# flo-stilz/Audio-Key-Estimation

Hardware: AMD Instinct MI355X
Metric: clips/s (15 s @ 22.05 kHz), HIP CQT + PitchClassNet forward (higher is better)
Workload: dtype f32 accumulation everywhere; pitch / semitone / layer-0 convolutions: f16 activations x f16 weights (per-channel power-of-two scaled) on MFMA, one product; last layer's pitch-class convolutions and heads: 3-term split-bf16 on MFMA (hi*hi + lo*hi + hi*lo); CQT filter bank: 3-term split-bf16 on MFMA

## Files before the change

audio-key-estimation_amd/csrc/pcnet.hip:

```cpp
#include <algorithm>
#include <cmath>
#include <cstdlib>
#include <cstring>
#include <map>
#include <string>
#include <vector>

#include "common.h"
#include "pcnet_kernels.h"
#include "pcnet_bwd_kernels.h"

using namespace ake_k;

namespace {

constexpr double kBnEps = 1e-5;
constexpr size_t kLdsBudget = 64 * 1024;
constexpr size_t kBfFragsPerConv = 14 * 2 * 64 + 64;

struct TensorSpec {
    std::string name;
    int64_t shape[4];
    int ndim;
};
// ... 412 lines not shown
    a.Tp = p2p_pitch(a.J);
    a.R = std::max(1, std::min(H, 8 * kP2pMT * 16 / a.J));
    auto lds_of = [&](int R) { return (static_cast<size_t>(R + 6) * a.Tp + (kP2pStreamB ? 0 : kBfFragsPerConv)) * sizeof(uint4); };
    while (a.R > 1 && lds_of(a.R) > 76 * 1024) --a.R;
    AKE_REQUIRE(lds_of(a.R) <= 150 * 1024, AKE_ERR_UNSUPPORTED, "conv %s: %d frames do not fit the bf16 kernel's LDS patch", name, T);
    a.n_row_tiles = (H + a.R - 1) / a.R;
    static ake::DeviceOnce attr_set;
    if (attr_set.need()) {
        AKE_HIP_CHECK(hipFuncSetAttribute(reinterpret_cast<const void*>(conv_p2p_f16_kernel<true, false>), hipFuncAttributeMaxDynamicSharedMemorySize, 150 * 1024));
        AKE_HIP_CHECK(hipFuncSetAttribute(reinterpret_cast<const void*>(conv_p2p_f16_kernel<false, false>), hipFuncAttributeMaxDynamicSharedMemorySize, 150 * 1024));
        AKE_HIP_CHECK(hipFuncSetAttribute(reinterpret_cast<const void*>(conv_p2p_f16_kernel<true, true>), hipFuncAttributeMaxDynamicSharedMemorySize, 150 * 1024));
        attr_set.mark();
    }
    dim3 grid(a.n_row_tiles, 1, batch), block(512);
    ake::ProfScope ps(name, s);
    AKE_REQUIRE(!nchw || oh, AKE_ERR_STATE, "conv %s: the assembling variant writes channels-last planes", name);
    if (nchw) hipLaunchKernelGGL((conv_p2p_f16_kernel<true, true>), grid, block, lds_of(a.R), s, a);
    else if (oh) hipLaunchKernelGGL((conv_p2p_f16_kernel<true, false>), grid, block, lds_of(a.R), s, a);
    else hipLaunchKernelGGL((conv_p2p_f16_kernel<false, false>), grid, block, lds_of(a.R), s, a);
    return AKE_OK;
}

int g_keep_taps = 0;

int device_cus() {
    static int n_cus = 0;
    if (!n_cus) {
        int dev = 0;
        if (hipGetDevice(&dev) != hipSuccess || hipDeviceGetAttribute(&n_cus, hipDeviceAttributeMultiprocessorCount, dev) != hipSuccess) n_cus = -1;
    }
    return n_cus;
}

int p2p_ps_rows(int H, int T, bool semi, int* plane_pos, size_t* lds) {
    if (T < 2 || (T & 1) || device_cus() < 8) return 0;
    const int J = T / 2, Tp = p2p_pitch(J);
    auto plane_of = [&](int R) { return ((R + 6) * Tp + 63) / 64 * 64; };
    auto lds_of = [&](int R) { return (static_cast<size_t>(2) * plane_of(R) + (semi ? 2 * 8 * kP2pMT * 16 * 2 : 8 * kP2pMT * kP2pPsStage)) * sizeof(uint4); };
    int R = std::max(1, std::min(H, 8 * kP2pMT * 16 / J));
    if (semi) R = R / 3 * 3;
    while (R >= (semi ? 3 : 1) && (lds_of(R) > 156 * 1024 || plane_of(R) / 64 > 8 * kP2pPieces)) R -= semi ? 3 : 1;
    if (R < (semi ? 3 : 1) || H < R + 6) return 0;
    if (semi && (H % 3 || (H / 3) % 12)) return 0;
    if (plane_pos) *plane_pos = plane_of(R);
    if (lds) *lds = lds_of(R);
    return R;
}

bool p2p_fuses_semi(const ake_pcnet* n, int i, int P, int T) {
    return !g_keep_taps && !n->cfg.p2pc_conv && !n->cfg.stay_sixth && i == n->cfg.num_layers - 1 && p2p_uses_f16(n, i, T) && static_cast<size_t>(i) < n->semi.size() && n->semi[i].bf_off >= 0 &&
           p2p_ps_rows(P, T, true, nullptr, nullptr) > 0;
}

enum class P2pIn : unsigned char {
    Planes,
    Src,
    SrcFramesMajor,
    SrcF16x4,
};
enum class P2pOut : unsigned char {
    Plane,
    Nchw,
    Semi,
    SemiFold,
};
struct P2pPsIo {
    P2pIn in = P2pIn::Planes;
    const unsigned short* planes = nullptr;
    Src src{};
    P2pOut out = P2pOut::Plane;
    unsigned short* plane = nullptr;
    float* dst = nullptr;
    int dst_ctot = 0;
    int fold_coff = 0;
// ... 61 lines not shown
        }
    }
    a.dst = io.dst; a.dst_clip_stride = static_cast<long long>(io.dst_ctot) * (semi ? H / 3 : H) * T; a.oh = io.plane;
    if (semi) { a.sfrag = n->bf_frags_dev + io.semi->bf_off; a.sbias = n->blob_dev + io.semi->b_off; }
    a.H = H; a.T = T; a.J = T / 2; a.Tp = p2p_pitch(a.J);
    a.n_row_tiles = g.n_row_tiles; a.n_tiles = g.n_tiles;
    if (io.out == P2pOut::SemiFold) {
        a.n_oct = g.n_oct; a.n_units = g.n_units;
        a.dst = io.dst + static_cast<long long>(io.fold_coff) * 12 * T;
        a.dst_clip_stride = static_cast<long long>(io.dst_ctot) * 12 * T;
    }
    static ake::DeviceOnce attr_set;
    if (attr_set.need()) {
        const void* fns[] = {reinterpret_cast<const void*>(conv_p2p_f16_ps_kernel<3, 0>),
                             reinterpret_cast<const void*>(conv_p2p_f16_ps_kernel<1, 0>), reinterpret_cast<const void*>(conv_p2p_f16_ps_kernel<1, 5>),
                             reinterpret_cast<const void*>(conv_p2p_f16_ps_kernel<1, 8>), reinterpret_cast<const void*>(conv_p2p_f16_ps_kernel<0, 0>),
                             reinterpret_cast<const void*>(conv_p2p_f16_ps_kernel<2, 0>), reinterpret_cast<const void*>(conv_p2p_f16_ps_kernel<1, 3>)};
        for (const void* f : fns) AKE_HIP_CHECK(hipFuncSetAttribute(f, hipFuncAttributeMaxDynamicSharedMemorySize, 160 * 1024));
        attr_set.mark();
    }
    dim3 grid(g.grid), block(512);
    ake::ProfScope ps(name, s);
    switch (io.out) {
        case P2pOut::SemiFold: hipLaunchKernelGGL((conv_p2p_f16_ps_kernel<3, 0>), grid, block, g.lds, s, a); break;
        case P2pOut::Semi: hipLaunchKernelGGL((conv_p2p_f16_ps_kernel<2, 0>), grid, block, g.lds, s, a); break;
        case P2pOut::Nchw: hipLaunchKernelGGL((conv_p2p_f16_ps_kernel<0, 0>), grid, block, g.lds, s, a); break;
        case P2pOut::Plane:
            if (io.in == P2pIn::Planes) hipLaunchKernelGGL((conv_p2p_f16_ps_kernel<1, 0>), grid, block, g.lds, s, a);
            else if (io.in == P2pIn::SrcF16x4) hipLaunchKernelGGL((conv_p2p_f16_ps_kernel<1, 3>), grid, block, g.lds, s, a);
            else if (a.c0 + a.c1 <= 5) hipLaunchKernelGGL((conv_p2p_f16_ps_kernel<1, 5>), grid, block, g.lds, s, a);
            else hipLaunchKernelGGL((conv_p2p_f16_ps_kernel<1, 8>), grid, block, g.lds, s, a);
            break;
    }
    return AKE_OK;
}

struct P2pX3Plan {
    bool ok = false;
    int R = 0, plane_pos = 0, n_row_tiles = 0, n_tiles = 0, grid = 0;
    size_t lds = 0;
};
P2pX3Plan p2p_f16x3_plan(int c0, int c1, int cout, int batch, int H, int T, bool dst16) {
    P2pX3Plan g;
    if (T < 2 || (T & 1) || c0 < 1 || c0 + c1 > 8 || cout > 8 || batch < 1) return g;
    const int n_cus = device_cus();
    if (n_cus < 8) return g;
    const int Tp = p2p_pitch(T / 2);
    auto plane_of = [&](int R) { return ((R + 6) * Tp + 63) / 64 * 64; };
    auto lds_of = [&](int R) { return (static_cast<size_t>(4) * plane_of(R) + 8 * kP2pMT * kP2pPsStage) * sizeof(uint4); };
    int R = std::max(1, std::min(H, 8 * kP2pMT * 16 / (T / 2)));
    while (R >= 1 && (lds_of(R) > 156 * 1024 || plane_of(R) > 3 * 512)) --R;
    if (R < 1 || H < R + 6) return g;
    if ((R * T) % 4 || (static_cast<long long>(H) * T) % 4 || (static_cast<long long>(cout) * H * T) % 4 || !dst16) return g;
    g.R = R; g.plane_pos = plane_of(R); g.lds = lds_of(R);
    g.n_row_tiles = (H + R - 1) / R;
    g.n_tiles = g.n_row_tiles * batch;
    g.grid = std::min(n_cus / 8 * 8, (g.n_tiles + 7) / 8 * 8);
    g.ok = true;
    return g;
}

int run_p2p_f16x3(const ake_pcnet* n, const P2pX3Plan& g, long long frag_off, const Src& src, const float* in_aff, const float* bias, int batch, int H, int T,
                  float* dst, int cout, double* stats, int stats_stride, hipStream_t s, const char* name, const unsigned int* in_amax = nullptr, bool lrelu = false) {
    AKE_REQUIRE(g.ok && frag_off >= 0 && src.ctot0 == 0, AKE_ERR_STATE, "conv %s: a convolution that does not qualify was sent to the f16 x 3 persistent kernel", name);
    AKE_REQUIRE(g.n_tiles == g.n_row_tiles * batch, AKE_ERR_STATE, "conv %s: the f16 x 3 persistent kernel was planned for another batch than these %d clips", name, batch);
    AKE_REQUIRE(!(reinterpret_cast<uintptr_t>(dst) & 15), AKE_ERR_STATE, "conv %s: the f16 x 3 persistent kernel was planned for 16-byte stores to an unaligned tensor", name);
// ... 335 lines not shown
            if (h == 2 && !c.genre) break;
            for (int j = 0; j + 1 < c.head_layers; ++j) {
                b->hst[h].push_back(cv.take<float>(hid));
                b->aff_hst[h].push_back(cv.take<float>(3 * 2 * n->final_ch));
            }
            b->g_map[h] = cv.take<float>(B * 12 * b->Tf);
        }
    }
    b->bytes = ake::align_up(cv.off, 256);
    return AKE_OK;
}

enum class L0Form : unsigned char { Generic, FusedValu, FusedMfma };
enum class PStack : unsigned char { Generic, F16x3, F16 };
enum class PcStack : unsigned char { Generic, F16x3, Bf16, Fused };
enum class HeadForm : unsigned char { Generic, Bf16First, Head1, Fused };

struct Layer0Plan {
    L0Form form = L0Form::Generic;
    int RP = 0, RPp = 0;
    size_t lds = 0;
};

struct Route {
    bool frames_major = false;
    Layer0Plan l0;
    bool psix_f16 = false;
    int chunk_clips[2] = {0, 0};
    struct Pitch {
        PStack stack = PStack::Generic;
        unsigned x3_convs = 0;
        struct PerChunk {
            P2pPsPlan first, mid, last;
            P2pX3Plan x3[2];
        } k[2];
    } p[4];
    PcStack pc = PcStack::Generic;
    unsigned pc_x3_convs = 0;
    HeadForm heads = HeadForm::Generic;
    bool genre_bf = false;
    bool heads_pool = false;
    int heads_mt = 0;
    int T1 = 0, T2 = 0, TpB = 0;
    size_t hf_lds = 0;

    int chunk_kind(int B) const { return B == chunk_clips[0] ? 0 : 1; }
};

Layer0Plan layer0_plan(const ake_pcnet* n, int T0, bool mel16, bool mel_fm) {
    const auto& c = n->cfg;
    const int P = c.pitches, NF = c.n_filters;
    Layer0Plan g;
    if (c.num_layers < 2 || c.resblock || c.denseblock || c.p2pc_conv || c.stay_sixth || NF < 2 || NF > 4 || c.conv_layers < 1 || c.conv_layers > 4 || c.kernel_size != 7 || P % 36 || T0 < 1) return g;
    const PackedConv& sp = n->semi[0];
    if (sp.cin != 1 || sp.co != 1) return g;
    bool mfma = c.precision == AKE_PRECISION_MIXED;
    for (int j = 0; j < c.conv_layers; ++j) {
        const PackedConv& pc = n->pc2pc[0][j];
        if (pc.co != 4 || pc.groups != 1 || pc.kh != 12 || pc.kw != 7 || pc.cout != NF || pc.cin != (j == 0 ? 1 : NF)) return g;
        mfma = mfma && pc.l0_off >= 0;
    }
    if (n->dims[1].prev_pc != NF) return g;
    g.RP = 4 * ((T0 + 3) / 4) + 8;
    g.RPp = (T0 + 8 + 1) / 2 * 2;
    const size_t lds_v = (static_cast<size_t>(9) * 12 * g.RP + static_cast<size_t>(P) * T0) * sizeof(float);
    if (lds_v > 150 * 1024 || (static_cast<long long>(P) * T0) % 4 || !mel16) return g;
// ... 14 lines not shown
    for (int i = 0; i < L; ++i) Tl[i] = i < 2 ? frames : Tl[i - 1] / c.time_pool_size;
    const int Tf = L > 1 ? Tl[L - 1] / c.time_pool_size : frames;
    if (batch < 1 || chunk < 1 || Tf < 1) return r;
    r.chunk_clips[0] = std::min(batch, chunk);
    r.chunk_clips[1] = batch > chunk ? batch % chunk : 0;

    if (!train && L > 1) r.l0 = layer0_plan(n, Tl[0], !(reinterpret_cast<uintptr_t>(mel) & 15), mel_fm);
    if (r.l0.form == L0Form::FusedMfma && !g_keep_taps && !c.pc2p_mem && n->dims[1].prev_p == 1 && p2p_uses_f16(n, 1, Tl[1])) {
        r.psix_f16 = true;
        for (int k = 0; k < 2 && r.psix_f16; ++k)
            if (r.chunk_clips[k])
                r.psix_f16 = p2p_ps_plan(P2pIn::SrcF16x4, 1, n->dims[1].prev_pc, P2pOut::Plane, n->dims[1].out_p, false, r.chunk_clips[k], c.pitches, Tl[1], ws16).ok;
    }

    const int P = c.stay_sixth ? c.pitches / 3 : c.pitches;
    int cp = 1;
    for (int i = 1; i < L && !c.denseblock && !c.resblock; ++i) {
        const LayerDims& d = n->dims[i];
        Route::Pitch& rp = r.p[i];
        const int Ti = Tl[i], c0 = cp, c1 = c.pc2p_mem ? 0 : d.prev_pc;
        if (!train && p2p_uses_f16(n, i, Ti)) {
            rp.stack = PStack::F16;
            const bool semi = p2p_fuses_semi(n, i, P, Ti);
            for (int k = 0; k < 2; ++k) {
                const int B = r.chunk_clips[k];
                if (!B) continue;
                const P2pIn in0 = (i == 1 && r.psix_f16) ? P2pIn::SrcF16x4 : ((mel_fm && i == 1) ? P2pIn::SrcFramesMajor : P2pIn::Src);
                rp.k[k].first = p2p_ps_plan(in0, c0, c1, P2pOut::Plane, d.out_p, false, B, P, Ti, ws16);
                rp.k[k].mid = p2p_ps_plan(P2pIn::Planes, 0, 0, P2pOut::Plane, d.out_p, false, B, P, Ti, ws16);
                P2pPsPlan& last = rp.k[k].last;
                if (semi) last = p2p_ps_plan(P2pIn::Planes, 0, 0, P2pOut::SemiFold, d.prev_pc + d.out_p, true, B, P, Ti, ws16);
                if (semi && !last.ok) last = p2p_ps_plan(P2pIn::Planes, 0, 0, P2pOut::Semi, d.out_p, true, B, P, Ti, ws16);
                if (!last.ok) last = p2p_ps_plan(P2pIn::Planes, 0, 0, P2pOut::Nchw, d.out_p, false, B, P, Ti, ws16);
            }
        } else if (!c.pc2p_mem && !c.stay_sixth && (train || (c.precision == AKE_PRECISION_F32X3 && !g_keep_taps))) {
            for (int k = 0; k < 2; ++k) {
                const int B = r.chunk_clips[k];
                if (!B) continue;
                rp.k[k].x3[0] = p2p_f16x3_plan(c0, c1, d.out_p, B, P, Ti, ws16);
                rp.k[k].x3[1] = p2p_f16x3_plan(d.out_p, 0, d.out_p, B, P, Ti, ws16);
            }
            for (int j = 0; j < c.conv_layers && j < 32; ++j)
                if ((train ? n->p2p_t[i][j] : n->p2p[i][j]).bf_off >= 0 && rp.k[0].x3[j > 0].ok) rp.x3_convs |= 1u << j;
            if (rp.x3_convs) rp.stack = PStack::F16x3;
        }
        cp = d.out_p;
    }
    r.frames_major = mel_fm && !train && L == 2 && !c.resblock && !c.denseblock && !c.pc2p_mem && !c.p2pc_conv && !c.stay_sixth && !c.local &&
                     batch <= chunk && r.l0.form == L0Form::FusedMfma && r.p[1].stack == PStack::F16 && r.p[1].k[0].first.ok;

    const int i = L - 1, Ti = Tl[i];
    if (!train && L > 1 && !c.denseblock && pc2pc_fuses(n, i, Ti)) r.pc = PcStack::Fused;
    else if (!train && pc2pc_uses_bf16(n, i, Ti)) r.pc = PcStack::Bf16;
    else if (train && L > 1 && !c.resblock && !c.denseblock) {
        for (int j = 0; j < c.conv_layers && j < 32; ++j)
            if (pc_f16x3_ok(n->pc2pc_t[i][j], Ti, true)) r.pc_x3_convs |= 1u << j;
        if (r.pc_x3_convs) r.pc = PcStack::F16x3;
    }

    const bool head_bf = !train && L > 1 && n->final_ch == 16 && c.head_layers >= 2 && n->head_key[0].bf_off >= 0 && n->head_tonic[0].bf_off >= 0 &&
                         Tf <= kPcBf16MaxFrames;
    if (!head_bf) return r;
    r.heads = HeadForm::Bf16First;
    r.T1 = Tf - (c.kernel_size - 1); r.T2 = r.T1 - (c.kernel_size - 1);
    const int T1 = r.T1, T2 = r.T2;
    if (!(c.head_layers == 2 && n->head_key[1].bf_off >= 0 && n->head_tonic[1].bf_off >= 0 && T2 > 0 && (12 * ((T2 + 15) / 16) + 15) / 16 <= kHead1MT)) return r;
// ... 1273 lines not shown
                {
                    ake::ProfScope ps("slice_channels_kernel", s);
                    hipLaunchKernelGGL(slice_channels_kernel, dim3(static_cast<unsigned>((total + 255) / 256)), dim3(256), 0, s, pcs,
                                       static_cast<long long>(ctot) * 12 * Ti, b.pcd[i], per_clip, total);
                }
                sdesc = Src{p_cur, cp, b.pcd[i], d.prev_pc, 12};
                if (train) {
                    if (i == 1) AKE_HIP_CHECK(hipMemcpyAsync(b.aff_p2pin[i], b.aff_semi[0], sizeof(float) * 3 * cp, hipMemcpyDeviceToDevice, s));
                    else identity(b.aff_p2pin[i], cp);
                    AKE_HIP_CHECK(hipMemcpyAsync(b.aff_p2pin[i] + 3 * cp, b.aff_cat[i], sizeof(float) * 3 * d.prev_pc, hipMemcpyDeviceToDevice, s));
                }
            }
            if (c.pc2p_mem) {
                const long long total = static_cast<long long>(B) * cp * P * Ti;
                ake::ProfScope ps("pc2p_mem_kernel", s);
                hipLaunchKernelGGL(pc2p_mem_kernel, dim3(static_cast<unsigned>((total + 255) / 256)), dim3(256), 0, s, p_cur, psix, b.pin[i], cp,
                                   d.prev_pc / cp, P, Ti, total, train ? b.aff_p2pin[i] + 3 * d.prev_p : nullptr);
                sdesc = Src{b.pin[i], cp, nullptr, 0, 0};
            }
            const float* in_aff = train ? b.aff_p2pin[i] : nullptr;
            float* out = nullptr;
            float* out_aff = nullptr;
            const Route::Pitch& rp = r.p[i];
            const Route::Pitch::PerChunk& rk = rp.k[r.chunk_kind(B)];
            P2pOut last_out = P2pOut::Nchw;
            if (c.resblock && train) {
                if ((rc = res_stack_train(n->p2p_t[i], m + "p2p.layer.", 0, sdesc, in_aff, B, P, Ti, b.pst[i], b.aff_pst[i], nullptr, 0, "conv_mfma_kernel/p2p")))
                    return rc;
                out = b.pst[i].back(); out_aff = b.aff_pst[i].back();
            } else if (c.resblock) {
                if ((rc = res_stack(n->p2p[i], 0, sdesc, B, P, Ti, b.pa[i], b.pb[i], nullptr, 0, "conv_mfma_kernel/p2p"))) return rc;
                out = b.pa[i];
            }
            for (int j = 0; j < c.conv_layers && !c.resblock; ++j) {
                out = train ? b.pst[i][j] : ((j & 1) ? b.pb[i] : b.pa[i]);
                out_aff = !train ? nullptr : b.aff_pst[i][j];
                if (rp.stack == PStack::F16) {
                    const bool last_conv = j == c.conv_layers - 1;
                    const P2pPsPlan& g = j == 0 ? rk.first : (last_conv ? rk.last : rk.mid);
                    P2pPsIo io;
                    io.in = g.in; io.out = g.out;
                    io.dst_ctot = d.out_p;
                    if (j > 0) io.planes = reinterpret_cast<const unsigned short*>(((j - 1) & 1) ? b.pb[i] : b.pa[i]);
                    else if (g.in == P2pIn::SrcF16x4)
                        io.src = Src{reinterpret_cast<const float*>(b.melh + static_cast<size_t>(c0) * P * Ti), 1,
                                     reinterpret_cast<const float*>(reinterpret_cast<const uint2*>(b.psix[1]) + static_cast<size_t>(c0) * 36 * Ti), d.prev_pc, 36};
                    else io.src = sdesc;
                    switch (g.out) {
                        case P2pOut::Plane: io.plane = reinterpret_cast<unsigned short*>(out); break;
                        case P2pOut::Nchw: io.dst = out; break;
                        case P2pOut::Semi: io.dst = out; io.semi = &n->semi[i]; break;
                        case P2pOut::SemiFold: io.dst = cat; io.dst_ctot = ctot; io.fold_coff = d.prev_pc; io.semi = &n->semi[i]; break;
                    }
                    if (last_conv) last_out = g.out;
                    AKE_REQUIRE(g.ok || g.in == P2pIn::Planes || g.in == P2pIn::Src, AKE_ERR_STATE,
                                "pcnet: the route promised an input form only the persistent pitch conv reads, for a chunk (%d clips) it does not take", B);
                    if (g.ok) rc = run_p2p_f16_ps(n, n->p2p[i][j], g, io, B, P, Ti, s, "conv_p2p_f16_kernel");
                    else rc = run_p2p_f16(n, n->p2p[i][j], io.planes, j == 0 ? &io.src : nullptr, B, P, Ti, io.dst, d.out_p, io.plane, s, "conv_p2p_f16_kernel");
                    if (rc) return rc;
                    continue;
                }
                if (rp.x3_convs >> j & 1) {
                    const PackedConv& px = train ? n->p2p_t[i][j] : n->p2p[i][j];
                    const int bn = train ? bn_of(m + "p2p.layer." + std::to_string(3 * j + 1)) : -1;
                    if ((rc = run_p2p_f16x3(n, rk.x3[j > 0], px.bf_off, sdesc, in_aff, n->blob_dev + px.b_off, B, P, Ti, out, d.out_p,
                                            train ? b.stats + 2 * n->bns[bn].ch_off : nullptr, train ? 2 * n->bn_channels : 0, s, "conv_p2p_f16x3_kernel/p2p", nullptr,
                                            !train)))
// ... 584 lines not shown
```

audio-key-estimation_amd/csrc/pcnet_kernels.h:

```cpp
#pragma once

#include <hip/hip_runtime.h>

#include "common.h"

namespace ake_k {

constexpr int TW = 4;
constexpr float kSlope = 0.01f;

struct ConvArgs {
    const float* src0;
    const float* src1;
    long long src0_clip_stride, src1_clip_stride;
    int c0, c1, h1;
    int H;
    int T_in;
    int T_out;
    int H_out;
    int py;
    int pad_l;
    int time_circ;
    const float* w;
    const float* bias;
// ... 679 lines not shown
#pragma unroll
            for (int i = 0; i < 4; ++i)
                if (pos[i] >= 0) oh[pos[i] * 8] = static_cast<unsigned short>(f16_bits(v[i]));
        } else {
#pragma unroll
            for (int i = 0; i < 4; ++i)
                if (pos[i] >= 0) od[pos[i]] = v[i];
        }
    }
}

struct P2pPsArgs {
    const unsigned short* xh;
    const float* p;
    const float* u;
    const uint2* uh;
    const unsigned int* ph;
    int c0, c1, h1;
    int p_fm;
    const uint4* bfrag;
    const float* bias;
    float* dst;
    long long dst_clip_stride;
    unsigned short* oh;
    const uint4* sfrag;
    const float* sbias;
    int H, T, R, J, Tp, n_row_tiles, n_tiles, plane_pos;
    int n_oct, n_units;
};

constexpr int kP2pPieces = 3;
constexpr int kP2pPsStage = 80;

template <int OUT, int NIN>
__global__ __launch_bounds__(512, ((NIN > 0 && NIN != 3) ? 2 : 4)) void conv_p2p_f16_ps_kernel(P2pPsArgs a) {
    constexpr bool OUT_CL = OUT == 1, OUT_SEMI = OUT == 2 || OUT == 3, OUT_FOLD = OUT == 3;
    constexpr bool IN_NCHW = NIN > 0;
    constexpr bool IN_UH = NIN == 3;
    constexpr int NV = IN_UH ? 1 : (IN_NCHW ? NIN : 1);
    extern __shared__ __attribute__((aligned(16))) uint4 lds4[];
    constexpr int MT = kP2pMT;
    const int lane = threadIdx.x & 63;
    const int wave = __builtin_amdgcn_readfirstlane(threadIdx.x >> 6);
    const int r16 = lane & 15, q = lane >> 4;
    const int Tp = a.Tp, J = a.J, T = a.T;
    f16_saturate_mode();
    const int nchunk = a.plane_pos >> 6;
    const int npos = (a.R + 6) * Tp;
    const int nwg = gridDim.x, per_xcd = nwg >> 3;
    const int first = (blockIdx.x & 7) * per_xcd + (blockIdx.x >> 3);
    int pk[kP2pPieces];
#pragma unroll
    for (int k = 0; k < kP2pPieces; ++k) {
        const int c = wave + 8 * k;
        int i = c * 64 + lane;
        i = i < npos ? i : npos - 1;
        const int rj = i / Tp, f = i - rj * Tp;
        pk[k] = (rj << 16) | wrap(f - 3, T);
    }
    auto issue_loads = [&](int tile, int buf) {
        const int clip = tile / a.n_row_tiles;
        const int y0 = (tile - clip * a.n_row_tiles) * a.R;
        const long long cbase = static_cast<long long>(clip) * a.H * T;
#pragma unroll
        for (int k = 0; k < kP2pPieces; ++k) {
            const int c = wave + 8 * k;
            if (c < nchunk) {
                int row = y0 - 3 + (pk[k] >> 16);
                row += row < 0 ? a.H : 0;
                row -= row >= a.H ? a.H : 0;
                const uint4* src = reinterpret_cast<const uint4*>(a.xh) + cbase + static_cast<long long>(row) * T + (pk[k] & 0xffff);
                uint4* dstl = lds4 + buf * a.plane_pos + c * 64;
                ake::lds_dma_16(src, static_cast<unsigned int>(reinterpret_cast<unsigned long long>(dstl)));
            }
        }
    };
    float vin[3][NV];
    uint2 vuh[3];
    unsigned int vw[3];
    int pn[3];
    if (IN_NCHW) {
#pragma unroll
        for (int k = 0; k < 3; ++k) {
            const int i = threadIdx.x + 512 * k;
            const int ic = i < npos ? i : npos - 1;
            const int rj = ic / Tp, f = ic - rj * Tp;
            pn[k] = (rj << 16) | wrap(f - 3, T);
        }
    }
    auto load_regs = [&](int tile) {
        const int clip = tile / a.n_row_tiles;
        const int y0 = (tile - clip * a.n_row_tiles) * a.R;
        const int ctot = a.c0 + a.c1;
        const float* const pb = a.p_fm ? a.p + static_cast<long long>(clip) * T * a.H : a.p + static_cast<long long>(clip) * a.c0 * a.H * T;
        const float* const ub = a.u + static_cast<long long>(clip) * a.c1 * a.h1 * T;
        const uint2* const uhb = IN_UH ? uniform_ptr(a.uh + static_cast<long long>(clip) * a.h1 * T) : nullptr;
#pragma unroll
        for (int k = 0; k < 3; ++k) {
            int row = y0 - 3 + (pn[k] >> 16);
            row += row < 0 ? a.H : 0;
            row -= row >= a.H ? a.H : 0;
            const int t = pn[k] & 0xffff;
            if (IN_UH) {
                vw[k] = uniform_ptr(a.ph + static_cast<long long>(clip) * a.H * T)[static_cast<unsigned int>(row * T + t)];
                vuh[k] = uhb[static_cast<unsigned int>((row % a.h1) * T + t)];
                continue;
            }
            const int poff = a.p_fm ? t * a.H + row : row * T + t;
            const int uoff = (row % a.h1) * T + t;
#pragma unroll
            for (int c = 0; c < NV; ++c) {
                const int cc = c < ctot ? c : ctot - 1;
                const float* const base = uniform_ptr(cc < a.c0 ? pb + static_cast<long long>(cc) * a.H * T : ub + static_cast<long long>(cc - a.c0) * a.h1 * T);
                vin[k][c] = base[static_cast<unsigned int>(cc < a.c0 ? poff : uoff)];
            }
        }
    };
    auto write_lds = [&](int buf) {
        uint4* const wH = lds4 + buf * a.plane_pos;
        const int ctot = a.c0 + a.c1;
#pragma unroll
        for (int k = 0; k < 3; ++k) {
            unsigned int hi[4] = {0, 0, 0, 0};
            typedef float f32x2w __attribute__((ext_vector_type(2)));
            if (IN_UH) {
                const unsigned int hb = vw[k] & 0xffffu;
                hi[0] = hb | (vuh[k].x << 16);
                hi[1] = (vuh[k].x >> 16) | (vuh[k].y << 16);
                hi[2] = (vuh[k].y >> 16) | (vw[k] & 0xffff0000u);
                hi[3] = hb;
                const int i = threadIdx.x + 512 * k;
                if (i < npos) wH[i] = make_uint4(hi[0], hi[1], hi[2], hi[3]);
                continue;
            }
#pragma unroll
            for (int c = 0; c < NV; c += 2) {
                const f32x2w v = {c < ctot ? vin[k][c] : 0.f, (c + 1 < NV && c + 1 < ctot) ? vin[k][c + 1 < NV ? c + 1 : c] : 0.f};
                hi[c >> 1] = __builtin_bit_cast(unsigned int, __builtin_convertvector(v, f16x2c));
            }
            if (NV <= kP2pSplit0 && ctot <= kP2pSplit0) {
                const _Float16 h0 = static_cast<_Float16>(vin[k][0]);
                hi[2] = (hi[2] & 0xffffu) | (f16_bits(vin[k][0] - static_cast<float>(h0)) << 16);
                hi[3] = static_cast<unsigned int>(__builtin_bit_cast(unsigned short, h0));
            }
            const int i = threadIdx.x + 512 * k;
            if (i < npos) wH[i] = make_uint4(hi[0], hi[1], hi[2], hi[3]);
        }
    };
    const int G = OUT_FOLD ? a.n_row_tiles / a.n_oct : 1;
    auto fold_tile = [&](int u, int o) { const int clip = u / G; return clip * a.n_row_tiles + o * G + (u - clip * G); };
    const int tile0 = OUT_FOLD ? (first < a.n_units ? fold_tile(first, 0) : -1) : (first < a.n_tiles ? first : -1);
    if (tile0 >= 0) {
        if (IN_NCHW) { load_regs(tile0); write_lds(0); }
        else issue_loads(tile0, 0);
    }
    uint4 breg[28];
#pragma unroll
    for (int i = 0; i < 28; ++i) breg[i] = a.bfrag[i * 64 + lane];
    int abase[MT];
#pragma unroll
    for (int mt = 0; mt < MT; ++mt) {
        int m = (wave * MT + mt) * 16 + r16;
        m = m < a.R * J ? m : a.R * J - 1;
        const int r = m / J, j = m - r * J;
        abase[mt] = r * Tp + 2 * j + q;
    }
    const int tau = r16 >> 3, co = r16 & 7;
    const float bias = a.bias[co];
    const float iscale = reinterpret_cast<const float*>(a.bfrag + kP2pFragScale)[co];
    uint4* const stage = lds4 + 2 * a.plane_pos + wave * (MT * kP2pPsStage);
    uint4* const opatch = lds4 + 2 * a.plane_pos;
    constexpr int kOP = 8 * MT * 16 * 2;
    typedef float f32x2e __attribute__((ext_vector_type(2)));
    long long prev_base = 0;
    int prev_mblk = 0;
    bool has_prev = false;
    auto store_pending = [&]() {
        if (OUT_CL) {
            static_assert(MT == 3, "the M-tiles leave as one pair and a single");
            const uint4 o01 = stage[(lane >> 5) * kP2pPsStage + (lane & 31)], o2 = stage[2 * kP2pPsStage + (lane & 31)];
            const int mb01 = (wave * MT + (lane >> 5)) * 16, mb2 = (wave * MT + 2) * 16, ml = (lane >> 1) & 15;
            uint4* const o = reinterpret_cast<uint4*>(a.oh) + prev_base + (lane & 31);
            if (mb01 + ml < prev_mblk) o[2 * mb01] = o01;
            if (lane < 32 && mb2 + ml < prev_mblk) o[2 * mb2] = o2;
            return;
        }
        uint4 outv[MT];
#pragma unroll
        for (int mt = 0; mt < MT; ++mt) outv[mt] = stage[mt * kP2pPsStage + (lane >> 3) * 9 + (lane & 7)];
#pragma unroll
        for (int mt = 0; mt < MT; ++mt) {
            const int mbase = (wave * MT + mt) * 16;
            {
                const int m = mbase + 2 * (lane & 7);
                float* o = a.dst + prev_base + static_cast<long long>(lane >> 3) * a.H * T + 2 * m;
                if (m + 1 < prev_mblk) *reinterpret_cast<uint4*>(o) = outv[mt];
                else if (m < prev_mblk) { o[0] = __uint_as_float(outv[mt].x); o[1] = __uint_as_float(outv[mt].y); }
            }
        }
    };
    auto epilogue = [&](const f32x4c (&acc)[MT], const f32x4c (&accl)[MT], int obuf) {
#pragma unroll
        for (int mt = 0; mt < MT; ++mt) {
            float v[4];
#pragma unroll
// ... 28 lines not shown
        sbias = a.sbias[co];
        siscale = reinterpret_cast<const float*>(a.sfrag + 6 * 64)[co];
        int ms = wave * 16 + r16;
        ms = ms < (a.R / 3) * J ? ms : (a.R / 3) * J - 1;
        const int srow = ms / J, sj = ms - srow * J;
        sbase = 3 * srow * T + wrap(2 * sj - 1 + q, T);
    }
    float smax[4] = {0.f, 0.f, 0.f, 0.f};
    auto semi_stage = [&](int obuf, long long base, int mblk, int oct) {
        const uint4* const oH = opatch + obuf * kOP;
        f32x4c sacc = {0.f, 0.f, 0.f, 0.f}, saccl = {0.f, 0.f, 0.f, 0.f};
#pragma unroll
        for (int dy = 0; dy < 3; ++dy) {
            const f16x8c ah = __builtin_bit_cast(f16x8c, oH[sbase + dy * T]);
            const f16x8c bh = __builtin_bit_cast(f16x8c, sreg[2 * dy]), bl = __builtin_bit_cast(f16x8c, sreg[2 * dy + 1]);
            sacc = __builtin_amdgcn_mfma_f32_16x16x32_f16(ah, bh, sacc, 0, 0, 0);
            if (kP2pProducts == 2) saccl = __builtin_amdgcn_mfma_f32_16x16x32_f16(ah, bl, saccl, 0, 0, 0);
        }
        const int S = OUT_FOLD ? 12 : a.H / 3;
        float* const o = a.dst + base + static_cast<long long>(co) * S * T + tau;
#pragma unroll
        for (int i = 0; i < 4; ++i) {
            const int m = wave * 16 + 4 * q + i;
            const float x = fmaf(kP2pProducts == 2 ? fmaf(saccl[i], kP2pLoInv, sacc[i]) : sacc[i], siscale, sbias);
            const float v = fmaxf(x, x * kSlope);
            if (!OUT_FOLD) {
                if (3 * m < mblk) o[2 * m] = v;
            } else {
                smax[i] = oct == 0 ? v : fmaxf(smax[i], v);
                if (oct == a.n_oct - 1 && 3 * m < mblk) o[2 * m] = smax[i];
            }
        }
    };
    const bool late = !OUT_SEMI && wave >= 4;
    f32x4c acc[MT], accl[MT];
#pragma unroll
    for (int mt = 0; mt < MT; ++mt) { acc[mt] = f32x4c{0.f, 0.f, 0.f, 0.f}; accl[mt] = f32x4c{0.f, 0.f, 0.f, 0.f}; }
    int cur = 0;
    int unit = first, oct = 0, prev_oct = 0;
    for (int tile = tile0; tile >= 0; cur ^= 1) {
        int next, n_unit = unit, n_oct_i = oct;
        if (OUT_FOLD) {
            if (++n_oct_i == a.n_oct) { n_oct_i = 0; n_unit += nwg; }
            next = n_unit < a.n_units ? fold_tile(n_unit, n_oct_i) : -1;
        } else next = tile + nwg < a.n_tiles ? tile + nwg : -1;
        __builtin_amdgcn_s_waitcnt(0x0F70);
        __syncthreads();
        const bool more = next >= 0;
        if (has_prev) {
            if (OUT_SEMI) semi_stage(cur ^ 1, prev_base, prev_mblk, prev_oct);
            else if (late) epilogue(acc, accl, 0);
        }
        const uint4* const pH = lds4 + cur * a.plane_pos;
#pragma unroll
        for (int mt = 0; mt < MT; ++mt) { acc[mt] = f32x4c{0.f, 0.f, 0.f, 0.f}; accl[mt] = f32x4c{0.f, 0.f, 0.f, 0.f}; }
#pragma unroll
        for (int ks = 0; ks < 14; ++ks) {
            if (ks == 2 && more) {
                if (IN_NCHW) load_regs(next);
                else issue_loads(next, cur ^ 1);
            }
            if (ks == 6 && !OUT_SEMI && has_prev) store_pending();
            const int dy = ks >> 1, h = ks & 1;
            const f16x8c bh = __builtin_bit_cast(f16x8c, breg[2 * ks]), bl = __builtin_bit_cast(f16x8c, breg[2 * ks + 1]);
            f16x8c ah[MT];
#pragma unroll
            for (int mt = 0; mt < MT; ++mt) ah[mt] = __builtin_bit_cast(f16x8c, pH[abase[mt] + dy * Tp + 4 * h]);
#pragma unroll
            for (int mt = 0; mt < MT; ++mt) acc[mt] = __builtin_amdgcn_mfma_f32_16x16x32_f16(ah[mt], bh, acc[mt], 0, 0, 0);
#pragma unroll
            for (int mt = 0; mt < MT; ++mt)
                if (kP2pProducts == 2) accl[mt] = __builtin_amdgcn_mfma_f32_16x16x32_f16(ah[mt], bl, accl[mt], 0, 0, 0);
        }
        if (!late) epilogue(acc, accl, cur);
        if (IN_NCHW && more) write_lds(cur ^ 1);
        {
            const int clip = tile / a.n_row_tiles;
            const int y0 = (tile - clip * a.n_row_tiles) * a.R;
            const int rows_here = a.H - y0 < a.R ? a.H - y0 : a.R;
            prev_mblk = rows_here * J;
            prev_base = OUT_CL ? static_cast<long long>(clip) * a.H * T + static_cast<long long>(y0) * T
                      : OUT_FOLD ? clip * a.dst_clip_stride + static_cast<long long>((y0 % 36) / 3) * T
                      : OUT_SEMI ? clip * a.dst_clip_stride + static_cast<long long>(y0 / 3) * T
                                 : clip * a.dst_clip_stride + static_cast<long long>(y0) * T;
            prev_oct = oct;
        }
        has_prev = true;
        tile = next; unit = n_unit; oct = n_oct_i;
    }
    if (has_prev) {
        if (OUT_SEMI) {
            __syncthreads();
            semi_stage(cur ^ 1, prev_base, prev_mblk, prev_oct);
        } else {
            if (late) epilogue(acc, accl, 0);
            store_pending();
        }
    }
}

struct P2pTrArgs {
    const float* p;
    const float* u;
    int c0, c1, h1;
    const float* in_aff;
    const uint4* bfrag;
    const float* bias;
    float* dst;
    long long dst_clip_stride;
    int cout;
    double* stats;
    int stats_stride;
    int H, T, R, J, Tp, n_row_tiles, n_tiles, plane_pos;
    const unsigned int* in_amax;
    int lrelu;
};

__global__ __launch_bounds__(512) void conv_p2p_f16x3_kernel(P2pTrArgs a) {
    extern __shared__ __attribute__((aligned(16))) uint4 lds4[];
    constexpr int MT = kP2pMT, NV = 8;
    const int lane = threadIdx.x & 63;
    const int wave = __builtin_amdgcn_readfirstlane(threadIdx.x >> 6);
    const int r16 = lane & 15, q = lane >> 4;
    const int Tp = a.Tp, J = a.J, T = a.T;
    const int npos = (a.R + 6) * Tp;
    const int nwg = gridDim.x, per_xcd = nwg >> 3;
    const int first = (blockIdx.x & 7) * per_xcd + (blockIdx.x >> 3);
    const int ctot = a.c0 + a.c1;
    float vin[3][NV];
    int pn[3];
#pragma unroll
// ... 1769 lines not shown
```

Measured before the change: 466,800.

## Fuse the f16 pitch conv stack into one per-clip 1024-thread launch

Adds a p2p_stack_kernel that runs all pitch-to-pitch convolutions of the last layer, including the semitone fold, inside one launch. Each workgroup owns one clip and walks every conv phase in turn, using workgroup barriers with release/acquire fences in place of kernel boundaries. The tile routine is templated on wave count and chaining so it can serve both the old multi-launch path and the new 16-wave path. The intent is to remove launch overhead and inter-kernel gaps. In exchange, parallelism is limited to one workgroup per clip, and the path only engages when the batch nearly fills the CUs.

```diff
diff --git a/audio-key-estimation_amd/csrc/pcnet.hip b/audio-key-estimation_amd/csrc/pcnet.hip
--- a/audio-key-estimation_amd/csrc/pcnet.hip
+++ b/audio-key-estimation_amd/csrc/pcnet.hip
@@ -468,14 +468,14 @@
     return n_cus;
 }
 
-int p2p_ps_rows(int H, int T, bool semi, int* plane_pos, size_t* lds) {
+int p2p_ps_rows(int H, int T, bool semi, int* plane_pos, size_t* lds, int nw = 8) {
     if (T < 2 || (T & 1) || device_cus() < 8) return 0;
     const int J = T / 2, Tp = p2p_pitch(J);
     auto plane_of = [&](int R) { return ((R + 6) * Tp + 63) / 64 * 64; };
-    auto lds_of = [&](int R) { return (static_cast<size_t>(2) * plane_of(R) + (semi ? 2 * 8 * kP2pMT * 16 * 2 : 8 * kP2pMT * kP2pPsStage)) * sizeof(uint4); };
-    int R = std::max(1, std::min(H, 8 * kP2pMT * 16 / J));
+    auto lds_of = [&](int R) { return (static_cast<size_t>(2) * plane_of(R) + (semi ? 2 * nw * kP2pMT * 16 * 2 : nw * kP2pMT * kP2pPsStage)) * sizeof(uint4); };
+    int R = std::max(1, std::min(H, nw * kP2pMT * 16 / J));
     if (semi) R = R / 3 * 3;
-    while (R >= (semi ? 3 : 1) && (lds_of(R) > 156 * 1024 || plane_of(R) / 64 > 8 * kP2pPieces)) R -= semi ? 3 : 1;
+    while (R >= (semi ? 3 : 1) && (lds_of(R) > 156 * 1024 || plane_of(R) / 64 > nw * kP2pPieces || (semi && nw == 16 && 36 % R))) R -= semi ? 3 : 1;
     if (R < (semi ? 3 : 1) || H < R + 6) return 0;
     if (semi && (H % 3 || (H / 3) % 12)) return 0;
     if (plane_pos) *plane_pos = plane_of(R);
@@ -603,6 +603,67 @@
             else hipLaunchKernelGGL((conv_p2p_f16_ps_kernel<1, 8>), grid, block, g.lds, s, a);
             break;
     }
+    return AKE_OK;
+}
+
+struct P2pStackPlan {
+    bool ok = false;
+    int n = 0;
+    int R[2] = {0, 0}, plane_pos[2] = {0, 0}, n_row_tiles[2] = {0, 0};
+    int n_oct = 0;
+    size_t lds = 0;
+};
+P2pStackPlan p2p_stack_plan(int convs, int c0, int c1, bool semi_frags, int batch, int H, int T) {
+    P2pStackPlan g;
+    const int n_cus = device_cus();
+    if (convs < 2 || convs > kP2pStackMax || c0 != 1 || c1 < 1 || c1 > 4 || !semi_frags || batch < 1 || batch > n_cus || 16 * (n_cus - batch) > n_cus) return g;
+    size_t lds[2] = {0, 0};
+    for (int f = 0; f < 2; ++f) {
+        g.R[f] = p2p_ps_rows(H, T, f == 1, &g.plane_pos[f], &lds[f], 16);
+        if (g.R[f] <= 0) return g;
+        g.n_row_tiles[f] = (H + g.R[f] - 1) / g.R[f];
+    }
+    if (H % 36 || 36 % g.R[1]) return g;
+    g.n_oct = H / 36;
+    g.lds = std::max(lds[0], lds[1]);
+    g.n = convs;
+    g.ok = true;
+    return g;
+}
+
+int run_p2p_stack(const ake_pcnet* n, const std::vector<PackedConv>& convs, const PackedConv& semi, const P2pStackPlan& g, const unsigned int* melh, const uint2* psix_h,
+                  int c1, unsigned short* const planes[], float* cat, int cat_ctot, int fold_coff, int batch, int H, int T, hipStream_t s, const char* name) {
+    AKE_REQUIRE(g.ok && g.n == static_cast<int>(convs.size()) && batch <= device_cus(), AKE_ERR_STATE,
+                "conv %s: the route sent a stack to the one-launch kernel that does not qualify for it", name);
+    AKE_REQUIRE(melh && psix_h && cat && semi.bf_off >= 0, AKE_ERR_STATE, "conv %s: the one-launch stack lacks a buffer", name);
+    P2pStackArgs sa;
+    std::memset(&sa, 0, sizeof(sa));
+    sa.n = g.n;
+    for (int j = 0; j < g.n; ++j) {
+        const bool fold = j == g.n - 1;
+        P2pPsArgs& a = sa.ph[j];
+        AKE_REQUIRE(fold || planes[j], AKE_ERR_STATE, "conv %s: the one-launch stack lacks a plane", name);
+        a.R = g.R[fold]; a.plane_pos = g.plane_pos[fold]; a.n_row_tiles = g.n_row_tiles[fold]; a.n_tiles = a.n_row_tiles * batch;
+        a.bfrag = n->bf_frags_dev + convs[j].bf_off; a.bias = n->blob_dev + convs[j].b_off;
+        a.H = H; a.T = T; a.J = T / 2; a.Tp = p2p_pitch(a.J);
+        if (j == 0) { a.ph = melh; a.uh = psix_h; a.c0 = 1; a.c1 = c1; a.h1 = 36; }
+        else a.xh = planes[j - 1];
+        if (!fold) a.oh = planes[j];
+        else {
+            a.sfrag = n->bf_frags_dev + semi.bf_off; a.sbias = n->blob_dev + semi.b_off;
+            a.n_oct = g.n_oct; a.n_units = batch * (36 / a.R);
+            a.dst = cat + static_cast<long long>(fold_coff) * 12 * T;
+            a.dst_clip_stride = static_cast<long long>(cat_ctot) * 12 * T;
+        }
+    }
+    static ake::DeviceOnce attr_set;
+    if (attr_set.need()) {
+        AKE_HIP_CHECK(hipFuncSetAttribute(reinterpret_cast<const void*>(p2p_stack_kernel), hipFuncAttributeMaxDynamicSharedMemorySize, 160 * 1024));
+        attr_set.mark();
+    }
+    dim3 grid(batch), block(1024);
+    ake::ProfScope ps(name, s);
+    hipLaunchKernelGGL(p2p_stack_kernel, grid, block, g.lds, s, sa);
     return AKE_OK;
 }
 
@@ -1004,6 +1065,7 @@
         unsigned x3_convs = 0;
         struct PerChunk {
             P2pPsPlan first, mid, last;
+            P2pStackPlan stack;
             P2pX3Plan x3[2];
         } k[2];
     } p[4];
@@ -1084,6 +1146,7 @@
                 if (semi) last = p2p_ps_plan(P2pIn::Planes, 0, 0, P2pOut::SemiFold, d.prev_pc + d.out_p, true, B, P, Ti, ws16);
                 if (semi && !last.ok) last = p2p_ps_plan(P2pIn::Planes, 0, 0, P2pOut::Semi, d.out_p, true, B, P, Ti, ws16);
                 if (!last.ok) last = p2p_ps_plan(P2pIn::Planes, 0, 0, P2pOut::Nchw, d.out_p, false, B, P, Ti, ws16);
+                if (in0 == P2pIn::SrcF16x4 && semi) rp.k[k].stack = p2p_stack_plan(c.conv_layers, c0, c1, true, B, P, Ti);
             }
         } else if (!c.pc2p_mem && !c.stay_sixth && (train || (c.precision == AKE_PRECISION_F32X3 && !g_keep_taps))) {
             for (int k = 0; k < 2; ++k) {
@@ -2423,7 +2486,18 @@
                 if ((rc = res_stack(n->p2p[i], 0, sdesc, B, P, Ti, b.pa[i], b.pb[i], nullptr, 0, "conv_mfma_kernel/p2p"))) return rc;
                 out = b.pa[i];
             }
-            for (int j = 0; j < c.conv_layers && !c.resblock; ++j) {
+            const bool one_launch = rp.stack == PStack::F16 && rk.stack.ok;
+            if (one_launch) {
+                unsigned short* planes[kP2pStackMax];
+                for (int j = 0; j < kP2pStackMax; ++j) planes[j] = reinterpret_cast<unsigned short*>((j & 1) ? b.pb[i] : b.pa[i]);
+                if ((rc = run_p2p_stack(n, n->p2p[i], n->semi[i], rk.stack, b.melh + static_cast<size_t>(c0) * P * Ti,
+                                        reinterpret_cast<const uint2*>(b.psix[1]) + static_cast<size_t>(c0) * 36 * Ti, d.prev_pc, planes, cat, ctot, d.prev_pc, B, P, Ti, s,
+                                        "conv_p2p_f16_kernel")))
+                    return rc;
+                out = ((c.conv_layers - 1) & 1) ? b.pb[i] : b.pa[i];
+                last_out = P2pOut::SemiFold;
+            }
+            for (int j = 0; j < c.conv_layers && !c.resblock && !one_launch; ++j) {
                 out = train ? b.pst[i][j] : ((j & 1) ? b.pb[i] : b.pa[i]);
                 out_aff = !train ? nullptr : b.aff_pst[i][j];
                 if (rp.stack == PStack::F16) {
diff --git a/audio-key-estimation_amd/csrc/pcnet_kernels.h b/audio-key-estimation_amd/csrc/pcnet_kernels.h
--- a/audio-key-estimation_amd/csrc/pcnet_kernels.h
+++ b/audio-key-estimation_amd/csrc/pcnet_kernels.h
@@ -735,8 +735,15 @@
 constexpr int kP2pPieces = 3;
 constexpr int kP2pPsStage = 80;
 
-template <int OUT, int NIN>
-__global__ __launch_bounds__(512, ((NIN > 0 && NIN != 3) ? 2 : 4)) void conv_p2p_f16_ps_kernel(P2pPsArgs a) {
+__device__ __forceinline__ void p2p_phase_sync() {
+    __builtin_amdgcn_s_waitcnt(0x0F70);
+    __builtin_amdgcn_fence(__ATOMIC_RELEASE, "workgroup");
+    __syncthreads();
+    __builtin_amdgcn_fence(__ATOMIC_ACQUIRE, "workgroup");
+}
+
+template <int OUT, int NIN, int NW, bool CHAIN>
+__device__ __forceinline__ void p2p_ps_tiles(const P2pPsArgs& a, const int first, const int step, const int limit) {
     constexpr bool OUT_CL = OUT == 1, OUT_SEMI = OUT == 2 || OUT == 3, OUT_FOLD = OUT == 3;
     constexpr bool IN_NCHW = NIN > 0;
     constexpr bool IN_UH = NIN == 3;
@@ -750,12 +757,10 @@
     f16_saturate_mode();
     const int nchunk = a.plane_pos >> 6;
     const int npos = (a.R + 6) * Tp;
-    const int nwg = gridDim.x, per_xcd = nwg >> 3;
-    const int first = (blockIdx.x & 7) * per_xcd + (blockIdx.x >> 3);
     int pk[kP2pPieces];
 #pragma unroll
     for (int k = 0; k < kP2pPieces; ++k) {
-        const int c = wave + 8 * k;
+        const int c = wave + NW * k;
         int i = c * 64 + lane;
         i = i < npos ? i : npos - 1;
         const int rj = i / Tp, f = i - rj * Tp;
@@ -767,7 +772,7 @@
         const long long cbase = static_cast<long long>(clip) * a.H * T;
 #pragma unroll
         for (int k = 0; k < kP2pPieces; ++k) {
-            const int c = wave + 8 * k;
+            const int c = wave + NW * k;
             if (c < nchunk) {
                 int row = y0 - 3 + (pk[k] >> 16);
                 row += row < 0 ? a.H : 0;
@@ -785,7 +790,7 @@
     if (IN_NCHW) {
 #pragma unroll
         for (int k = 0; k < 3; ++k) {
-            const int i = threadIdx.x + 512 * k;
+            const int i = threadIdx.x + 64 * NW * k;
             const int ic = i < npos ? i : npos - 1;
             const int rj = ic / Tp, f = ic - rj * Tp;
             pn[k] = (rj << 16) | wrap(f - 3, T);
@@ -832,7 +837,7 @@
                 hi[1] = (vuh[k].x >> 16) | (vuh[k].y << 16);
                 hi[2] = (vuh[k].y >> 16) | (vw[k] & 0xffff0000u);
                 hi[3] = hb;
-                const int i = threadIdx.x + 512 * k;
+                const int i = threadIdx.x + 64 * NW * k;
                 if (i < npos) wH[i] = make_uint4(hi[0], hi[1], hi[2], hi[3]);
                 continue;
             }
@@ -846,17 +851,20 @@
                 hi[2] = (hi[2] & 0xffffu) | (f16_bits(vin[k][0] - static_cast<float>(h0)) << 16);
                 hi[3] = static_cast<unsigned int>(__builtin_bit_cast(unsigned short, h0));
             }
-            const int i = threadIdx.x + 512 * k;
+            const int i = threadIdx.x + 64 * NW * k;
             if (i < npos) wH[i] = make_uint4(hi[0], hi[1], hi[2], hi[3]);
         }
     };
     const int G = OUT_FOLD ? a.n_row_tiles / a.n_oct : 1;
     auto fold_tile = [&](int u, int o) { const int clip = u / G; return clip * a.n_row_tiles + o * G + (u - clip * G); };
-    const int tile0 = OUT_FOLD ? (first < a.n_units ? fold_tile(first, 0) : -1) : (first < a.n_tiles ? first : -1);
-    if (tile0 >= 0) {
-        if (IN_NCHW) { load_regs(tile0); write_lds(0); }
-        else issue_loads(tile0, 0);
-    }
+    const int tile0 = first < limit ? (OUT_FOLD ? fold_tile(first, 0) : first) : -1;
+    auto first_patch = [&]() {
+        if (tile0 >= 0) {
+            if (IN_NCHW) { load_regs(tile0); write_lds(0); }
+            else issue_loads(tile0, 0);
+        }
+    };
+    if (!CHAIN) first_patch();
     uint4 breg[28];
 #pragma unroll
     for (int i = 0; i < 28; ++i) breg[i] = a.bfrag[i * 64 + lane];
@@ -873,7 +881,7 @@
     const float iscale = reinterpret_cast<const float*>(a.bfrag + kP2pFragScale)[co];
     uint4* const stage = lds4 + 2 * a.plane_pos + wave * (MT * kP2pPsStage);
     uint4* const opatch = lds4 + 2 * a.plane_pos;
-    constexpr int kOP = 8 * MT * 16 * 2;
+    constexpr int kOP = NW * MT * 16 * 2;
     typedef float f32x2e __attribute__((ext_vector_type(2)));
     long long prev_base = 0;
     int prev_mblk = 0;
@@ -968,7 +976,8 @@
             }
         }
     };
-    const bool late = !OUT_SEMI && wave >= 4;
+    if (CHAIN) { p2p_phase_sync(); first_patch(); }
+    const bool late = !OUT_SEMI && wave >= NW / 2;
     f32x4c acc[MT], accl[MT];
 #pragma unroll
     for (int mt = 0; mt < MT; ++mt) { acc[mt] = f32x4c{0.f, 0.f, 0.f, 0.f}; accl[mt] = f32x4c{0.f, 0.f, 0.f, 0.f}; }
@@ -977,9 +986,9 @@
     for (int tile = tile0; tile >= 0; cur ^= 1) {
         int next, n_unit = unit, n_oct_i = oct;
         if (OUT_FOLD) {
-            if (++n_oct_i == a.n_oct) { n_oct_i = 0; n_unit += nwg; }
-            next = n_unit < a.n_units ? fold_tile(n_unit, n_oct_i) : -1;
-        } else next = tile + nwg < a.n_tiles ? tile + nwg : -1;
+            if (++n_oct_i == a.n_oct) { n_oct_i = 0; n_unit += step; }
+            next = n_unit < limit ? fold_tile(n_unit, n_oct_i) : -1;
+        } else next = tile + step < limit ? tile + step : -1;
         __builtin_amdgcn_s_waitcnt(0x0F70);
         __syncthreads();
         const bool more = next >= 0;
@@ -1033,6 +1042,35 @@
             store_pending();
         }
     }
+}
+
+template <int OUT, int NIN>
+__global__ __launch_bounds__(512, ((NIN > 0 && NIN != 3) ? 2 : 4)) void conv_p2p_f16_ps_kernel(P2pPsArgs a) {
+    const int nwg = gridDim.x, per_xcd = nwg >> 3;
+    const int first = (blockIdx.x & 7) * per_xcd + (blockIdx.x >> 3);
+    p2p_ps_tiles<OUT, NIN, 8, false>(a, first, nwg, OUT == 3 ? a.n_units : a.n_tiles);
+}
+
+constexpr int kP2pStackMax = 4;
+struct P2pStackArgs {
+    P2pPsArgs ph[kP2pStackMax];
+    int n;
+};
+
+__global__ __launch_bounds__(1024) void p2p_stack_kernel(P2pStackArgs s) {
+    const int clip = blockIdx.x;
+    {
+        const int first = clip * s.ph[0].n_row_tiles;
+        p2p_ps_tiles<1, 3, 16, false>(s.ph[0], first, 1, first + s.ph[0].n_row_tiles);
+    }
+    for (int j = 1; j < s.n - 1; ++j) {
+        const P2pPsArgs& a = s.ph[j];
+        const int first = clip * a.n_row_tiles;
+        p2p_ps_tiles<1, 0, 16, true>(a, first, 1, first + a.n_row_tiles);
+    }
+    const P2pPsArgs& a = s.ph[s.n - 1];
+    const int G = a.n_row_tiles / a.n_oct;
+    p2p_ps_tiles<3, 0, 16, true>(a, clip * G, 1, clip * G + G);
 }
 
 struct P2pTrArgs {
```

Result: faster. 482,900, median of 6 (+3.4%).
